# wustl-cig/FLAIR

Measured on AMD Instinct MI355X. Metric: restored frames/sec at 256x256, 16-frame clip, 250-step DDIM, higher is better.
Workload: dtype bf16

## Files before the change

### flair_amd/csrc/conv.hip

```cpp
#include <type_traits>

#include "common.h"
#include "mfma_tile.h"

namespace {

struct ConvArgs {
    const void* x[4];
    int segC[4];
    int segLd[4];
    int nseg;
    const void* w;
    const float* bias;
    const void* res0;
    const void* res1;
    int res0Ld, res1Ld;
    void* y;
    int yLd;
    int T, H, W;
    int KT, KH, KW;
    int Cout, CinTot;
    int act;
    float outScale;
    long P;
// ... 958 lines not shown
            for (int jj = 0; jj < 2; ++jj) {
                const int cofs = i * 32 + 16 * jj;
                if (tl.co0 + cofs >= a.Cout) continue;
                const bool lane_ok = tl.co0 + cofs + cl < a.Cout;
                float bv[8];
                {
                    const float4 b0 = *reinterpret_cast<const float4*>(bl + cofs);
                    const float4 b1 = *reinterpret_cast<const float4*>(bl + cofs + 4);
                    bv[0] = b0.x; bv[1] = b0.y; bv[2] = b0.z; bv[3] = b0.w; bv[4] = b1.x; bv[5] = b1.y; bv[6] = b1.z; bv[7] = b1.w;
                }
#pragma unroll
                for (int j = 0; j < RPW; ++j) {
                    float v[8];
#pragma unroll
                    for (int e = 0; e < 4; ++e) {
                        const auto sw2 = __builtin_amdgcn_permlane32_swap(__float_as_uint(acc[j][i][8 * jj + e]),
                                                                          __float_as_uint(acc[j][i][8 * jj + 4 + e]), false, false);
                        v[e] = __uint_as_float(sw2[0]) + bv[e];
                        v[4 + e] = __uint_as_float(sw2[1]) + bv[4 + e];
                    }
                    if constexpr (ACT == 0) {
#pragma unroll
                        for (int e = 0; e < 8; ++e) v[e] = fmaxf(v[e], v[e] * slope);
                    } else if constexpr (ACT == 1) {
                        dcn_offset_act<8>(v, tl.co0 + cofs + cl, a.actParam, a.actPeriod);
                    } else {
#pragma unroll
                        for (int e = 0; e < 8; ++e) v[e] = silu_f(v[e]);
                    }
                    const long ro = (long)j * W;
                    if (r0b && lane_ok) add_piece<E>(v, r0b + ro * a.res0Ld + cofs);
                    if (r1b && lane_ok) add_piece<E>(v, r1b + ro * a.res1Ld + cofs);
#pragma unroll
                    for (int e = 0; e < 8; ++e) v[e] *= scale;
                    if (!lane_ok) continue;
                    Vec16<E>::store(yb + ro * a.yLd + cofs, v);
                }
            }
    };
    auto epilogue = [&](const DmaTile& tl, int biasSlot) {
        const bool res = a.res0 || a.res1;
        auto go = [&](auto actTag) {
            if constexpr (RPW == 1) {
                epilogue_plain_as(tl, biasSlot, actTag);
            } else {
                if (res) epilogue_as(tl, biasSlot, actTag, std::true_type{});
                else epilogue_as(tl, biasSlot, actTag, std::false_type{});
            }
        };
        if (a.act == FLAIR_ACT_DCN_OFFSETS) go(std::integral_constant<int, 1>{});
        else if (a.act == FLAIR_ACT_SILU) go(std::integral_constant<int, 2>{});
        else if (RPW >= 2 && a.act == FLAIR_ACT_NONE && a.outScale == 1.f) go(std::integral_constant<int, 3>{});
        else go(std::integral_constant<int, 0>{});
    };

    DmaTile cur, nxt;
    int iCur = 0, iNxt = 0;
    if (!tile_at(0, cur)) return;
    nxt = cur;
    Walk wk;
    walk_first(nxt.t, wk);
    setup_tile(nxt);
    float4 biasReg = make_float4(0.f, 0.f, 0.f, 0.f);
    bool biasPending = false;
    auto bias_request = [&](const DmaTile& tl) {
        if (tid < 16) {
            const int bco = tl.co0 + 4 * tid;
            biasReg = (a.bias && bco < a.Cout) ? *reinterpret_cast<const float4*>(a.bias + bco) : make_float4(0.f, 0.f, 0.f, 0.f);
            if (a.fbias && bco < a.Cout) {
                const float* fb = a.fbias + (long)tl.t * a.fbiasLd + bco;
                biasReg.x += fb[0]; biasReg.y += fb[1]; biasReg.z += fb[2]; biasReg.w += fb[3];
            }
        }
        biasPending = true;
    };
    auto bias_commit = [&](int slot_) {
        if (tid < 16) *reinterpret_cast<float4*>(smem + BIAS_OFF + (slot_ & 1) * 256 + 16 * tid) = biasReg;
        biasPending = false;
    };
    bias_request(nxt);
    bias_commit(0);
    const bool res0any = a.res0 || a.res1;
    int remIssue = chunks_of(nxt.t);
    int remCompute = remIssue;
    bool more = true;
    int stage = 0;
    issue(nxt, wk, 0);
    walk_next(nxt.t, wk);
    --remIssue;
    asm volatile("s_waitcnt vmcnt(0)" ::: "memory");
    __syncthreads();
    zero_acc();
    while (true) {
        if (more && remIssue == 0) {
            ++iNxt;
            more = tile_at(iNxt, nxt);
            if (more) {
                walk_first(nxt.t, wk);
                setup_tile(nxt);
                remIssue = chunks_of(nxt.t);
                bias_request(nxt);
            }
        }
        if (more) {
            issue(nxt, wk, stage ^ 1);
            walk_next(nxt.t, wk);
            --remIssue;
        }
        compute(stage);
        if (biasPending) bias_commit(iNxt);
        bool storesInFlight = false;
        if (--remCompute == 0) {
            epilogue(cur, iCur);
            storesInFlight = RPW >= 2 ? !a.res1 : cur.co0 + 64 <= a.Cout && !res0any;
            ++iCur;
            if (!tile_at(iCur, cur)) break;
            remCompute = chunks_of(cur.t);
            zero_acc();
        }
        if (storesInFlight) {
            asm volatile("s_waitcnt vmcnt(%0)" ::"n"(4 * RPW) : "memory");
        } else {
            asm volatile("s_waitcnt vmcnt(0)" ::: "memory");
        }
        __syncthreads();
        stage ^= 1;
    }
}

template <int RPW>
__global__ __launch_bounds__(512, 2) void conv3x3_dma_kernel(ConvArgs a, int nTiles, int tilesPerXcd) {
    prefetch_kernargs<sizeof(ConvArgs) + 8>();
    conv3x3_dma_body<RPW>(a, nTiles, tilesPerXcd);
}

template <int RPW>
int launch_dma(const ConvArgs& a0, hipStream_t s) {
    constexpr int NW = 8, NSTAGE = 2, TH = NW * RPW;
    ConvArgs a = a0;
    a.nCoTiles = cdiv(a.Cout, 64);
    a.tFast = a.KT == 3 && a.T > 1;
    const int nTiles = a.T * (a.H / TH) * (a.W / 32) * a.nCoTiles;
    const int nCu = flair_cu_count();
    int grid = nTiles < nCu ? (nTiles + 7) / 8 * 8 : nCu / 8 * 8;
    if (grid < 8) grid = 8;
    const int tilesPerXcd = (nTiles + 7) / 8;
    constexpr int HALO_INSTR = ((TH + 2) * 34 + 15) / 16;
    const size_t lds = NSTAGE * (size_t)(HALO_INSTR + 36) * 1024 + NW * 1024 + 512;
    static LdsAttrOnce attr;
    {
        const hipError_t e = flair_max_lds_once(attr, reinterpret_cast<const void*>(&conv3x3_dma_kernel<RPW>));
        FLAIR_CHECK(e == hipSuccess, "flair_conv_nhwc: hipFuncSetAttribute: %s", hipGetErrorString(e));
    }
    hipLaunchKernelGGL(conv3x3_dma_kernel<RPW>, dim3(grid), dim3(64 * NW), lds, s, a, nTiles, tilesPerXcd);
    FLAIR_LAUNCH_CHECK();
    return FLAIR_OK;
}


__global__ __launch_bounds__(512, 2) void conv_frame_kernel(ConvArgs a) {
    prefetch_kernargs<sizeof(ConvArgs)>();
    using E = bf16_t;
    constexpr int NW = 8, HWP = 34;
    constexpr int HINSTR = 22, HIMG = HINSTR * 1024, WINSTR = 36, SLOT = WINSTR * 1024;
    constexpr int HR = 3, WR = 2;
    constexpr int RING = HR * HIMG, BIAS = RING + WR * SLOT;
    constexpr int NH = (HINSTR + NW - 1) / NW, NWS = (WINSTR + NW - 1) / NW;
    extern __shared__ __attribute__((aligned(16))) char smem[];
    const int tid = threadIdx.x, lane = tid & 63;
    const int wave = __builtin_amdgcn_readfirstlane(tid >> 6);
    const int lr = lane & 31, lh = lane >> 5;
    const int lrow = lane >> 2, lchunk = lane & 3;
    const int tilesW = a.W / 32, perFrame = tilesW * (a.H / 8);
    const int bid = xcd_remap(blockIdx.x, gridDim.x);
    const int t = bid / perFrame, tile = bid - t * perFrame;
    const int h0 = (tile / tilesW) * 8, w0 = (tile % tilesW) * 32;
    const int nS = a.CinTot / 32;

    const u32x4_t wdesc = make_desc(a.w, a.wBytes);
    const u32x4_t bdesc = make_desc(a.bias, a.bias ? (unsigned)a.Cout * 4u : 0u);
    dma16(bdesc, (unsigned)(lane * 16), (unsigned)BIAS);
    unsigned hpix[NH], hpiece[NH];
#pragma unroll
    for (int i = 0; i < NH; ++i) dma_halo_coords((wave * NH + i) % HINSTR, lrow, lchunk, 10, h0, w0, a.H, a.W, hpix[i], hpiece[i]);
    unsigned wlane[NWS];
#pragma unroll
    for (int i = 0; i < NWS; ++i) {
        const int id = (wave * NWS + i) % WINSTR;
        const int row = id * 16 + lrow, tap9 = row >> 6, co = row & 63;
        wlane[i] = co < a.Cout ? (unsigned)((co * 9 + tap9) * a.CinTot) * 2u + (unsigned)((lchunk ^ ((co >> 2) & 3)) << 4) : FLAIR_OOB;
    }
    int hseg = 0, hcb = 0;
    auto issue_halo = [&](int slot) {
        const unsigned ld = (unsigned)a.segLd[hseg] * 2u;
        const u32x4_t xdesc = make_desc(reinterpret_cast<const char*>(a.x[hseg]) + (size_t)t * a.H * a.W * ld, a.segBytes[hseg]);
        const unsigned cofs = (unsigned)(hcb * 64);
#pragma unroll
        for (int i = 0; i < NH; ++i) {
            const int k = (wave * NH + i) % HINSTR;
            dma16(xdesc, hpix[i] == 0xffffffffu ? FLAIR_OOB : hpix[i] * ld + cofs + hpiece[i], (unsigned)(slot * HIMG + k * 1024));
        }
        if (++hcb * 32 >= a.segC[hseg]) {
            hcb = 0;
            ++hseg;
        }
    };
    auto issue_w = [&](int s_) {
#pragma unroll
        for (int i = 0; i < NWS; ++i) {
            const int id = (wave * NWS + i) % WINSTR;
            dma16(wdesc, wlane[i] == FLAIR_OOB ? FLAIR_OOB : wlane[i] + (unsigned)(s_ * 64), (unsigned)(RING + (s_ % WR) * SLOT + id * 1024));
        }
    };
    issue_halo(0);
    issue_w(0);
    if (nS > 1) {
        issue_halo(1);
        issue_w(1);
    }
    if (nS > 2) issue_halo(2);

    unsigned aoff[2], boff[3][2];
    dma_frag_offsets(lr, lh, wave * HWP, aoff, boff);
    f32x16 acc[2];
    auto compute = [&](int wslot, int hslot) { dma_tap_loop(smem + RING + wslot * SLOT, smem + hslot * HIMG, aoff, boff, acc, dma_no_hook{}); };

    const long prow = ((long)t * a.H + h0 + wave) * a.W + w0;
    const unsigned yLdB = (unsigned)a.yLd * 2u, r0LdB = (unsigned)a.res0Ld * 2u, r1LdB = (unsigned)a.res1Ld * 2u;
    const __amdgpu_buffer_rsrc_t yd = make_rsrc(reinterpret_cast<char*>(a.y) + prow * a.yLd * 2, (unsigned)a.W * yLdB);
    const __amdgpu_buffer_rsrc_t r0d = make_rsrc(a.res0 ? reinterpret_cast<const char*>(a.res0) + prow * a.res0Ld * 2 : nullptr, a.res0 ? (unsigned)a.W * r0LdB : 0u);
    const __amdgpu_buffer_rsrc_t r1d = make_rsrc(a.res1 ? reinterpret_cast<const char*>(a.res1) + prow * a.res1Ld * 2 : nullptr, a.res1 ? (unsigned)a.W * r1LdB : 0u);
    uint4 r0v[4], r1v[4];
#pragma unroll
    for (int g = 0; g < 4; ++g) r0v[g] = r1v[g] = make_uint4(0u, 0u, 0u, 0u);

    for (int s_ = 0; s_ < nS; ++s_) {
        if (s_ + 1 >= nS) asm volatile("s_waitcnt vmcnt(0)" ::: "memory");
        else if (s_ == 0 && nS > 2) asm volatile("s_waitcnt vmcnt(%0)" ::"n"(2 * NH + NWS) : "memory");
        else if (s_ == 0) asm volatile("s_waitcnt vmcnt(%0)" ::"n"(NH + NWS) : "memory");
        else asm volatile("s_waitcnt vmcnt(%0)" ::"n"(NH) : "memory");
        __builtin_amdgcn_s_barrier();
        if (s_ == 0) {
            const float* sb = reinterpret_cast<const float*>(smem + BIAS);
#pragma unroll
            for (int cf = 0; cf < 2; ++cf)
#pragma unroll
                for (int g = 0; g < 4; ++g) {
                    const float4 bq = *reinterpret_cast<const float4*>(sb + cf * 32 + 8 * g + 4 * lh);
                    acc[cf][4 * g] = bq.x; acc[cf][4 * g + 1] = bq.y; acc[cf][4 * g + 2] = bq.z; acc[cf][4 * g + 3] = bq.w;
                }
        }
        if (s_ >= 1 && s_ + 1 < nS) issue_w(s_ + 1);
        if (s_ >= 1 && s_ + 2 < nS) issue_halo((s_ + 2) % 3);
        if (s_ + 1 == nS) {
            if (a.res0) {
#pragma unroll
                for (int g = 0; g < 4; ++g) r0v[g] = buf_load16(r0d, 16 * g + 8 * lh < a.Cout ? (unsigned)lr * r0LdB + (unsigned)(32 * g + 16 * lh) : FLAIR_OOB);
            }
            if (a.res1) {
#pragma unroll
                for (int g = 0; g < 4; ++g) r1v[g] = buf_load16(r1d, 16 * g + 8 * lh < a.Cout ? (unsigned)lr * r1LdB + (unsigned)(32 * g + 16 * lh) : FLAIR_OOB);
            }
        }
        compute(s_ % WR, s_ % HR);
    }

    const float slope = leaky_slope(a.act);
    const float scale = a.outScale;
#pragma unroll
    for (int cf = 0; cf < 2; ++cf)
#pragma unroll
        for (int jj = 0; jj < 2; ++jj) {
            const int g = 2 * cf + jj;
            float v[8];
            acc_octet(acc[cf], jj, v);
            leaky_act(v, slope);
            add_piece<E>(v, r0v[g]);
            add_piece<E>(v, r1v[g]);
#pragma unroll
            for (int e = 0; e < 8; ++e) v[e] *= scale;
            store_piece(yd, pack_piece<E>(v), 16 * g + 8 * lh < a.Cout ? (unsigned)lr * yLdB + (unsigned)(32 * g + 16 * lh) : FLAIR_OOB);
        }
}

static bool frame_kernel_ok(const ConvArgs& a) {
    if (a.esz != 2 || a.KT != 1 || a.KH != 3 || a.KW != 3 || a.stride != 1 || a.fbias || a.Cout > 64 || a.Cout % 8 || a.W % 32 || a.H % 8) return false;
    if (!(a.act == FLAIR_ACT_NONE || a.act == FLAIR_ACT_RELU || a.act == FLAIR_ACT_LRELU01 || a.act == FLAIR_ACT_LRELU02)) return false;
    if (a.tapShift || a.reflect || a.CinTot % 32 || a.CinTot < 32) return false;
    for (int i = 0; i < a.nseg; ++i)
        if (a.segC[i] % 32) return false;
    return true;
}

static int launch_frame(const ConvArgs& a, hipStream_t s) {
    constexpr size_t lds = (3 * 22 + 2 * 36) * 1024 + 1024;
    static LdsAttrOnce attr;
    const hipError_t e = flair_max_lds_once(attr, reinterpret_cast<const void*>(&conv_frame_kernel));
    FLAIR_CHECK(e == hipSuccess, "flair_conv_nhwc: hipFuncSetAttribute: %s", hipGetErrorString(e));
    hipLaunchKernelGGL(conv_frame_kernel, dim3(a.T * (a.H / 8) * (a.W / 32)), dim3(512), lds, s, a);
    FLAIR_LAUNCH_CHECK();
    return FLAIR_OK;
}

template <typename E, int TC, int TP, int WC, int WP, int PD, int KWID>
__global__ __launch_bounds__(256) void conv_igemm_kernel(ConvArgs a) {
    prefetch_kernargs<sizeof(ConvArgs)>();
    constexpr int BKE = Mma<E>::BKE * KWID;
    constexpr int ROWB = 64 * KWID;
    constexpr int CPR = 4 * KWID;
    constexpr int RPP = 256 / CPR;
    constexpr int VEC = ET<E>::VEC;
    constexpr int FC = TC / WC / 32;
    constexpr int FP = TP / WP / 32;
    constexpr int XR = TP / RPP;
    constexpr int WR = TC / RPP;
    static_assert(WC * WP == 4 && FC >= 1 && FP >= 1 && XR >= 1 && WR >= 1, "tile");

    extern __shared__ __attribute__((aligned(16))) char smem[];
    constexpr int BUF = (TC + TP) * ROWB;
    auto loff = [](int row, int chunk) { return KWID == 1 ? lds_off(row, chunk) : row * 128 + ((chunk ^ ((row >> 1) & 7)) << 4); };

    const int tid = threadIdx.x;
    const int lane = tid & 63, wave = __builtin_amdgcn_readfirstlane(tid >> 6);
    const int wc = wave / WP, wp = wave % WP;

    const int bid = xcd_remap(blockIdx.x, gridDim.x);
    const int coTile = bid % a.nCoTiles;
    const int pixTile = bid / a.nCoTiles;
    const long p0 = (long)pixTile * TP;
    const int co0 = coTile * TC;

    const int chunk = tid % CPR;
    const int srow = tid / CPR;
    int xt[XR], xh[XR], xw[XR];
    bool xvalid[XR];
#pragma unroll
    for (int i = 0; i < XR; ++i) {
        long p = p0 + srow + RPP * i;
        xvalid[i] = p < a.P;
        if (!xvalid[i]) p = 0;
        int w_ = (int)(p % a.W);
        long q = p / a.W;
        xw[i] = w_;
        xh[i] = (int)(q % a.H);
        xt[i] = (int)(q / a.H);
    }
    const int taps = a.KT * a.KH * a.KW;
    const int pt = a.KT / 2, ph = a.KH / 2, pw = a.KW / 2;
    const int tFirst = (int)(p0 / ((long)a.H * a.W));
    const int tileFrames = (int)((TP + (long)a.H * a.W - 1) / ((long)a.H * a.W)) + 1;

    uint4 xreg[PD][XR], wreg[PD][WR];

    const int nkAll = taps * (a.CinTot / BKE);
    const int ks0 = (int)((long)blockIdx.y * nkAll / a.splitK);
    const int ks1 = (int)((long)(blockIdx.y + 1) * nkAll / a.splitK);
    int tap = ks0 / (a.CinTot / BKE), seg = 0, cb = ks0 % (a.CinTot / BKE), segOff = 0;
    while (cb * BKE >= a.segC[seg]) {
        cb -= a.segC[seg] / BKE;
        segOff += a.segC[seg];
        ++seg;
    }
    int dw = tap % a.KW - pw, dh = (tap / a.KW) % a.KH - ph, dt = tap / (a.KW * a.KH) - pt;

    const __amdgpu_buffer_rsrc_t wrs = make_rsrc(a.w, a.wBytes);
    constexpr unsigned ESZ = sizeof(E);
    auto issue_loads = [&](int set) {
        const int ld = a.segLd[seg];
        int fb = tFirst + dt;
        fb = fb < 0 ? 0 : (fb >= a.T ? a.T - 1 : fb);
        int nfr = a.T - fb;
        if (nfr > tileFrames) nfr = tileFrames;
        const size_t frameBytes = (size_t)a.Hin * a.Win * ld * ESZ;
        const __amdgpu_buffer_rsrc_t xr =
            make_rsrc(reinterpret_cast<const char*>(a.x[seg]) + fb * frameBytes, (unsigned)(nfr * frameBytes));
        const int coff = cb * BKE + chunk * VEC;
#pragma unroll
        for (int i = 0; i < XR; ++i) {
            const int t2 = xt[i] + dt;
            int h2 = xh[i] * a.stride + dh + a.tapShift, w2 = xw[i] * a.stride + dw + a.tapShift;
            if (a.reflect) {
                h2 = h2 < 0 ? -h2 : (h2 >= a.Hin ? 2 * a.Hin - 2 - h2 : h2);
                w2 = w2 < 0 ? -w2 : (w2 >= a.Win ? 2 * a.Win - 2 - w2 : w2);
            }
            const bool ok = xvalid[i] && (unsigned)t2 < (unsigned)a.T && (unsigned)h2 < (unsigned)a.Hin &&
                            (unsigned)w2 < (unsigned)a.Win;
            const unsigned off = ok ? (unsigned)((((t2 - fb) * a.Hin + h2) * a.Win + w2) * ld + coff) * ESZ : FLAIR_OOB;
            xreg[set][i] = buf_load16(xr, off);
        }
        const unsigned kofs = (unsigned)(tap * a.CinTot + segOff + coff) * ESZ;
#pragma unroll
        for (int j = 0; j < WR; ++j) {
            const int n = co0 + srow + RPP * j;
            wreg[set][j] = buf_load16(wrs, n < a.Cout ? (unsigned)(n * taps * a.CinTot) * ESZ + kofs : FLAIR_OOB);
        }
    };
    auto advance = [&]() {
        ++cb;
        if (cb * BKE >= a.segC[seg]) {
            cb = 0;
            segOff += a.segC[seg];
            ++seg;
            if (seg >= a.nseg) {
                seg = 0;
                segOff = 0;
                ++tap;
                ++dw;
                if (dw > pw) {
                    dw = -pw;
                    ++dh;
                    if (dh > ph) {
                        dh = -ph;
                        ++dt;
                    }
                }
            }
        }
    };
    auto write_lds = [&](int buf, int set) {
        char* base = smem + buf * BUF;
#pragma unroll
        for (int j = 0; j < WR; ++j)
            *reinterpret_cast<uint4*>(base + loff(srow + RPP * j, chunk)) = wreg[set][j];
#pragma unroll
        for (int i = 0; i < XR; ++i)
            *reinterpret_cast<uint4*>(base + TC * ROWB + loff(srow + RPP * i, chunk)) = xreg[set][i];
    };

    f32x16 acc[FC][FP];
#pragma unroll
    for (int i = 0; i < FC; ++i)
#pragma unroll
        for (int j = 0; j < FP; ++j)
#pragma unroll
            for (int r = 0; r < 16; ++r) acc[i][j][r] = 0.f;

    const int nk = ks1 - ks0;
    const int lr = lane & 31, lh = lane >> 5;

#pragma unroll
    for (int u = 0; u < PD; ++u)
        if (u < nk) {
            issue_loads(u);
            advance();
        }
    write_lds(0, 0);
    __syncthreads();

    for (int ks = 0; ks < nk; ks += PD) {
#pragma unroll
        for (int u = 0; u < PD; ++u) {
            const int k = ks + u;
            if (k >= nk) break;
            const int cur = k & 1;
            if (k + PD < nk) {
                issue_loads(u);
                advance();
            }
            const char* wb = smem + cur * BUF;
            const char* xb = wb + TC * ROWB;
#pragma unroll
            for (int sp = 0; sp < KWID; ++sp) {
                uint4 af[FC][2], bfr[FP][2];
#pragma unroll
                for (int i = 0; i < FC; ++i) {
                    const int row = wc * (TC / WC) + i * 32 + lr;
                    af[i][0] = *reinterpret_cast<const uint4*>(wb + loff(row, 4 * sp + Mma<E>::chunk(0, lh)));
                    af[i][1] = *reinterpret_cast<const uint4*>(wb + loff(row, 4 * sp + Mma<E>::chunk(1, lh)));
                }
#pragma unroll
                for (int j = 0; j < FP; ++j) {
                    const int row = wp * (TP / WP) + j * 32 + lr;
                    bfr[j][0] = *reinterpret_cast<const uint4*>(xb + loff(row, 4 * sp + Mma<E>::chunk(0, lh)));
                    bfr[j][1] = *reinterpret_cast<const uint4*>(xb + loff(row, 4 * sp + Mma<E>::chunk(1, lh)));
                }
#pragma unroll
                for (int i = 0; i < FC; ++i)
#pragma unroll
                    for (int j = 0; j < FP; ++j) Mma<E>::run(af[i], bfr[j], acc[i][j]);
            }
            if (k + 1 < nk) write_lds(cur ^ 1, (u + 1) % PD);
            __syncthreads();
        }
    }

    if (a.splitK > 1) {
#pragma unroll
        for (int j = 0; j < FP; ++j) {
            const long p = p0 + wp * (TP / WP) + j * 32 + lr;
            if (p >= a.P) continue;
#pragma unroll
            for (int i = 0; i < FC; ++i)
#pragma unroll
                for (int g = 0; g < 4; ++g) {
                    const int co = co0 + wc * (TC / WC) + i * 32 + 8 * g + 4 * lh;
                    if (co < a.Cout)
                        *reinterpret_cast<float4*>(a.part + ((long)blockIdx.y * a.P + p) * a.Cout + co) =
                            make_float4(acc[i][j][4 * g], acc[i][j][4 * g + 1], acc[i][j][4 * g + 2],
                                        acc[i][j][4 * g + 3]);
                }
        }
        return;
    }
    if ((a.Cout & 7) == 0 && ((uintptr_t)a.y & 15) == 0 && (a.yLd * (int)sizeof(E)) % 16 == 0 &&
        (!a.res0 || (((uintptr_t)a.res0 & 15) == 0 && (a.res0Ld * (int)sizeof(E)) % 16 == 0)) &&
        (!a.res1 || (((uintptr_t)a.res1 & 15) == 0 && (a.res1Ld * (int)sizeof(E)) % 16 == 0))) {
        auto run = [&](auto actTag) {
            igemm_epilogue<E, decltype(actTag)::value, FC, FP>(a, acc, p0 + wp * (TP / WP), co0 + wc * (TC / WC), lr, lh);
        };
        if (a.act == FLAIR_ACT_DCN_OFFSETS) run(std::integral_constant<int, 1>{});
        else if (a.act == FLAIR_ACT_SILU) run(std::integral_constant<int, 2>{});
        else if (a.act == FLAIR_ACT_GELU) run(std::integral_constant<int, 3>{});
        else run(std::integral_constant<int, 0>{});
        return;
    }
#pragma unroll
    for (int j = 0; j < FP; ++j) {
        const long p = p0 + wp * (TP / WP) + j * 32 + lr;
        if (p >= a.P) continue;
#pragma unroll
        for (int i = 0; i < FC; ++i)
#pragma unroll
            for (int g = 0; g < 4; ++g)
                store_quad<E>(a, p, co0 + wc * (TC / WC) + i * 32 + 8 * g + 4 * lh, acc[i][j][4 * g],
                              acc[i][j][4 * g + 1], acc[i][j][4 * g + 2], acc[i][j][4 * g + 3]);
    }
}

template <typename E>
__global__ void conv_splitk_reduce_kernel(ConvArgs a) {
    const unsigned cq = (unsigned)(a.Cout / 4);
    const unsigned quads = (unsigned)a.P * cq;
    const size_t slice = (size_t)a.P * a.Cout;
    for (unsigned i = blockIdx.x * blockDim.x + threadIdx.x; i < quads; i += gridDim.x * blockDim.x) {
        const unsigned p = i / cq;
        const int co = (int)(i - p * cq) * 4;
        const float* src = a.part + (size_t)p * a.Cout + co;
        float4 s = make_float4(0.f, 0.f, 0.f, 0.f);
        int k = 0;
        for (; k + 4 <= a.splitK; k += 4) {
            float4 v[4];
#pragma unroll
            for (int u = 0; u < 4; ++u) v[u] = *reinterpret_cast<const float4*>(src + (size_t)(k + u) * slice);
#pragma unroll
            for (int u = 0; u < 4; ++u) {
                s.x += v[u].x; s.y += v[u].y; s.z += v[u].z; s.w += v[u].w;
            }
        }
        for (; k < a.splitK; ++k) {
            const float4 v = *reinterpret_cast<const float4*>(src + (size_t)k * slice);
            s.x += v.x; s.y += v.y; s.z += v.z; s.w += v.w;
        }
        store_quad<E>(a, p, co, s.x, s.y, s.z, s.w);
    }
}

template <typename E, int TC, int TP, int WC, int WP, int PD, int KWID>
int launch_pd(const ConvArgs& a0, hipStream_t s) {
    ConvArgs a = a0;
    a.nPixTiles = cdiv(a.P, TP);
    a.nCoTiles = cdiv(a.Cout, TC);
    const int grid = a.nPixTiles * a.nCoTiles;
    const size_t lds = 2 * (TC + TP) * 64 * KWID;
    hipLaunchKernelGGL((conv_igemm_kernel<E, TC, TP, WC, WP, PD, KWID>), dim3(grid, a.splitK), dim3(256), lds, s, a);
    FLAIR_LAUNCH_CHECK();
    if (a.splitK > 1) {
        hipLaunchKernelGGL(conv_splitk_reduce_kernel<E>, dim3(grid_for(a.P * (a.Cout / 4), 256, 2048)), dim3(256), 0, s, a);
        FLAIR_LAUNCH_CHECK();
    }
    return FLAIR_OK;
}

template <typename E, int TC, int TP, int WC, int WP>
int launch(const ConvArgs& a, hipStream_t s) {
    if constexpr (sizeof(E) == 2) {
        bool ok = true;
        for (int i = 0; i < a.nseg; ++i) ok = ok && a.segC[i] % 64 == 0;
        if (ok) return launch_pd<E, TC, TP, WC, WP, 2, 2>(a, s);
    }
    return launch_pd<E, TC, TP, WC, WP, 4, 1>(a, s);
}

enum ConvVariant {
    IGEMM_128x128 = 0,
    IGEMM_64x128 = 1,
    IGEMM_64x64 = 2,
    HALO_8 = 3,
    HALO_4 = 4,
    HALO_2 = 5,
    HALO_KS_8 = 6,
    HALO_KS_4 = 7,
    DMA_CLIP = 8,
    DMA_FRAME = 9,
};

int choose_split(const ConvArgs& a, ConvVariant variant) {
    if (variant > IGEMM_64x64) return 1;
    const int maxBlocks = variant == IGEMM_128x128 ? 512 : 1024, maxSplit = 16;
    const int tc = variant == IGEMM_128x128 ? 128 : 64, tp = variant == IGEMM_64x64 ? 64 : 128;
    const int bke = 64 / (a.wBytes && a.CinTot ? (int)(a.wBytes / ((unsigned long long)a.Cout * a.KT * a.KH * a.KW * a.CinTot)) : 2);
    const long nk = (long)a.KT * a.KH * a.KW * (a.CinTot / bke);
    const long tiles = (long)cdiv(a.P, tp) * cdiv(a.Cout, tc);
    if (tiles >= 384 || nk < 32) return 1;
    long s = maxBlocks / tiles;
    if (s > maxSplit) s = maxSplit;
    if (s > nk / 8) s = nk / 8;
    return s < 1 ? 1 : (int)s;
}

ConvVariant choose_variant(const ConvArgs& a) {
    if (!a.reflect && a.stride == 1 && a.KH == 3 && a.KW == 3 && a.W % 32 == 0 && a.H >= 2) {
        const long per = (long)a.T * (a.W / 32) * cdiv(a.Cout, 64);
        const bool ks = a.Cout % 8 == 0;
        if (a.esz == 2 && ks && a.act != FLAIR_ACT_GELU && a.H % 16 == 0 && per * cdiv(a.H, 8) > 256 && per * (a.H / 16) >= 192) return DMA_CLIP;
        const bool dmaOk = a.esz == 2 && ks && a.act != FLAIR_ACT_GELU;
        if (per * cdiv(a.H, 8) >= 256) return ks && per * cdiv(a.H, 8) <= 256 ? (dmaOk && a.H % 8 == 0 ? DMA_FRAME : HALO_KS_8) : HALO_8;
        if (per * cdiv(a.H, 4) >= 256) return ks && per * cdiv(a.H, 4) <= 256 ? HALO_KS_4 : HALO_4;
        return HALO_2;
    }
    const long tiles128 = (long)cdiv(a.P, 128) * cdiv(a.Cout, 128);
    if (a.Cout > 64 && tiles128 >= 512) return IGEMM_128x128;
    if (a.Cout >= 128 && a.P >= 1024 && tiles128 <= 64 && (long)a.KT * a.KH * a.KW * a.CinTot >= 2304) return IGEMM_128x128;
    const long tiles64x128 = (long)cdiv(a.P, 128) * cdiv(a.Cout, 64);
    if (tiles64x128 >= 512) return IGEMM_64x128;
    return IGEMM_64x64;
}

template <typename E>
int dispatch(const ConvArgs& a0, hipStream_t s) {
    ConvArgs a = a0;
    const ConvVariant variant = choose_variant(a);
    a.splitK = a.part ? choose_split(a, variant) : 1;
    switch (variant) {
        case IGEMM_128x128: return launch<E, 128, 128, 2, 2>(a, s);
        case IGEMM_64x128: return launch<E, 64, 128, 1, 4>(a, s);
        case IGEMM_64x64: return launch<E, 64, 64, 2, 2>(a, s);
        case HALO_8: return launch_halo<E, 8>(a, s);
        case HALO_4: return launch_halo<E, 4>(a, s);
        case HALO_KS_8: return launch_halo_ks<E, 8>(a, s);
        case HALO_KS_4: return launch_halo_ks<E, 4>(a, s);
        case DMA_CLIP: return launch_dma<2>(a, s);
        case DMA_FRAME:
            if (frame_kernel_ok(a)) return launch_frame(a, s);
            return launch_dma<1>(a, s);
        case HALO_2: break;
    }
    return launch_halo<E, 2>(a, s);
}

}

extern "C" int flair_conv_variant(const flair_conv_params* p);

static void fill_geometry(ConvArgs& a, const flair_conv_params* p) {
    a.stride = p->stride > 1 ? p->stride : 1;
    a.Hin = p->H; a.Win = p->W;
    a.T = p->T; a.KT = p->KT; a.KH = p->KH; a.KW = p->KW; a.Cout = p->Cout;
    a.reflect = p->reflect_pad ? 1 : 0;
    a.act = p->act;
    a.H = (p->H + a.stride - 1) / a.stride;
    a.W = (p->W + a.stride - 1) / a.stride;
    a.P = (long)p->T * a.H * a.W;
    a.CinTot = 0;
    for (int i = 0; i < p->nseg && i < 4; ++i) a.CinTot += p->seg_c[i];
    const int esz = p->dtype == FLAIR_BF16 ? 2 : 4;
    a.esz = esz;
    a.wBytes = (unsigned)((unsigned long long)p->Cout * p->KT * p->KH * p->KW * a.CinTot * esz);
}

extern "C" size_t flair_conv_workspace_bytes(const flair_conv_params* p) {
    if (!p) return 0;
    ConvArgs a{};
    fill_geometry(a, p);
    const int split = choose_split(a, choose_variant(a));
    return split > 1 ? (size_t)split * a.P * a.Cout * sizeof(float) : 0;
}

extern "C" int flair_conv_nhwc(const flair_conv_params* p, const void* const* x, const void* w,
                               const float* bias, const float* frame_bias, const void* res0, const void* res1,
                               void* y, void* workspace, size_t workspace_bytes, hipStream_t stream) {
    FLAIR_CHECK(p && x && w && y, "flair_conv_nhwc: null argument");
    FLAIR_CHECK_DTYPE("flair_conv_nhwc", p->dtype);
    FLAIR_CHECK(p->nseg >= 1 && p->nseg <= 4, "flair_conv_nhwc: nseg %d not in 1..4", p->nseg);
    FLAIR_CHECK(p->T > 0 && p->H > 0 && p->W > 0 && p->Cout > 0, "flair_conv_nhwc: empty shape");
    FLAIR_CHECK((p->KT & 1) && (p->KH & 1) && (p->KW & 1), "flair_conv_nhwc: kernel taps must be odd");
    FLAIR_CHECK(p->Cout % 4 == 0, "flair_conv_nhwc: Cout %d must be a multiple of 4", p->Cout);
    const int bke = p->dtype == FLAIR_BF16 ? 32 : 16;
    const int esz = p->dtype == FLAIR_BF16 ? 2 : 4;
    ConvArgs a{};
    fill_geometry(a, p);
    for (int i = 0; i < p->nseg; ++i) {
        FLAIR_CHECK(x[i], "flair_conv_nhwc: segment %d is null", i);
        FLAIR_CHECK(p->seg_c[i] > 0 && p->seg_c[i] % bke == 0,
                    "flair_conv_nhwc: segment %d has %d channels; must be a multiple of %d", i, p->seg_c[i], bke);
        FLAIR_CHECK(p->seg_ld[i] >= p->seg_c[i] && (p->seg_ld[i] * esz) % 16 == 0 &&
                        ((uintptr_t)x[i]) % 16 == 0,
                    "flair_conv_nhwc: segment %d stride/alignment", i);
        a.x[i] = x[i];
        a.segC[i] = p->seg_c[i];
        a.segLd[i] = p->seg_ld[i];
        const unsigned long long bytes = (unsigned long long)p->H * p->W * p->seg_ld[i] * esz;
        FLAIR_CHECK(bytes < 0x40000000ull, "flair_conv_nhwc: one frame of segment %d spans %llu bytes (limit 1 GiB)",
                    i, bytes);
        a.segBytes[i] = (unsigned)bytes;
    }
    {
        const unsigned long long wb = (unsigned long long)p->Cout * p->KT * p->KH * p->KW * a.CinTot * esz;
        FLAIR_CHECK(wb < 0x80000000ull, "flair_conv_nhwc: weights span %llu bytes (limit 2 GiB)", wb);
    }
    const int gran = (p->dtype == FLAIR_BF16 && p->Cout % 8 != 0) ? 8 : 16;
    FLAIR_CHECK(p->y_ld >= p->Cout && (p->y_ld * esz) % gran == 0 && ((uintptr_t)y) % 16 == 0,
                "flair_conv_nhwc: output stride/alignment (y_ld = %d: >= Cout = %d, a multiple of %d bytes; y 16-byte aligned)",
                p->y_ld, p->Cout, gran);
    FLAIR_CHECK(!res0 || (p->res_ld[0] >= p->Cout && (p->res_ld[0] * esz) % gran == 0 && ((uintptr_t)res0) % gran == 0),
                "flair_conv_nhwc: res0 stride/alignment (res_ld = %d: >= Cout = %d; stride and pointer multiples of %d bytes)",
                p->res_ld[0], p->Cout, gran);
    FLAIR_CHECK(!res1 || (p->res_ld[1] >= p->Cout && (p->res_ld[1] * esz) % gran == 0 && ((uintptr_t)res1) % gran == 0),
                "flair_conv_nhwc: res1 stride/alignment (res_ld = %d: >= Cout = %d; stride and pointer multiples of %d bytes)",
                p->res_ld[1], p->Cout, gran);
    FLAIR_CHECK(((uintptr_t)w) % 16 == 0, "flair_conv_nhwc: weight alignment");
    FLAIR_CHECK(!bias || ((uintptr_t)bias) % 16 == 0, "flair_conv_nhwc: bias alignment");
    a.nseg = p->nseg;
    a.w = w;
    a.bias = bias;
    a.fbias = frame_bias;
    a.fbiasLd = p->frame_bias_ld;
    FLAIR_CHECK(!frame_bias || p->frame_bias_ld >= p->Cout, "flair_conv_nhwc: frame_bias_ld");
    {
        const unsigned long long hw = (unsigned long long)p->H * p->W * esz;
        FLAIR_CHECK(hw * p->y_ld < 0x40000000ull && (!res0 || hw * p->res_ld[0] < 0x40000000ull) && (!res1 || hw * p->res_ld[1] < 0x40000000ull),
                    "flair_conv_nhwc: one frame of the output / a residual spans more than 1 GiB");
    }
    a.res0 = res0;
    a.res1 = res1;
    a.res0Ld = p->res_ld[0];
    a.res1Ld = p->res_ld[1];
    a.y = y;
    a.yLd = p->y_ld;
    a.actParam = p->act_param;
    a.actPeriod = p->act_period;
    FLAIR_CHECK(p->act != FLAIR_ACT_DCN_OFFSETS || (p->act_period > 0 && p->act_period % 24 == 0),
                "flair_conv_nhwc: FLAIR_ACT_DCN_OFFSETS needs act_period = 3 * deform_groups (multiple of 24), got %d",
                p->act_period);
    a.outScale = p->out_scale;
    FLAIR_CHECK(a.stride == 1 || a.stride == 2, "flair_conv_nhwc: stride %d unsupported", p->stride);
    FLAIR_CHECK(!p->asym_pad || (a.stride == 2 && a.KH == a.KW && a.KT == 1 && p->H % 2 == 0 && p->W % 2 == 0),
                "flair_conv_nhwc: asym_pad needs a square 2-D stride-2 kernel on even frames");
    a.tapShift = p->asym_pad ? a.KH / 2 : 0;
    FLAIR_CHECK(!p->reflect_pad || (!p->asym_pad && a.KT == 1 && p->H > a.KH / 2 && p->W > a.KW / 2),
                "flair_conv_nhwc: reflect_pad needs a 2-D kernel smaller than the frame");
    a.part = nullptr;
    a.splitK = 1;

    const size_t need = flair_conv_workspace_bytes(p);
    if (workspace && need > 0 && workspace_bytes >= need) {
        FLAIR_CHECK(((uintptr_t)workspace) % 16 == 0, "flair_conv_nhwc: workspace alignment");
        a.part = reinterpret_cast<float*>(workspace);
    }
    if (p->dtype == FLAIR_BF16) return dispatch<bf16_t>(a, stream);
    return dispatch<float>(a, stream);
}

extern "C" int flair_conv_variant(const flair_conv_params* p) {
    if (!p) return -1;
    ConvArgs a{};
    fill_geometry(a, p);
    return choose_variant(a);
}
```

Measured before the change: 0.8652.

## Add intra-workgroup K-group split to implicit-GEMM conv with LDS reduction

Adds a KG template parameter so one workgroup runs 256*KG threads, each 256-thread group handling its own slice of the K loop in separate LDS staging buffers. The partial accumulators are then reduced through LDS before the epilogue. A new plan function picks KG=2 for 128x128 tiles and KG=4 for 64x64 tiles in bf16, cutting the cross-block split-K factor and with it the fp32 workspace traffic and reduce kernel. The change also raises the K threshold for the small-tile 128x128 path in bf16. The cost is more LDS per workgroup, which can lower occupancy, plus extra barriers and an LDS reduction step.

```diff
diff --git a/flair_amd/csrc/conv.hip b/flair_amd/csrc/conv.hip
--- a/flair_amd/csrc/conv.hip
+++ b/flair_amd/csrc/conv.hip
@@ -1284,8 +1284,9 @@
     return FLAIR_OK;
 }
 
-template <typename E, int TC, int TP, int WC, int WP, int PD, int KWID>
-__global__ __launch_bounds__(256) void conv_igemm_kernel(ConvArgs a) {
+template <typename E, int TC, int TP, int WC, int WP, int PD, int KWID, int KG>
+__global__ __launch_bounds__(256 * KG) void conv_igemm_kernel(ConvArgs a) {
+    static_assert(KG == 1 || KG == 2 || KG == 4, "K groups");
     prefetch_kernargs<sizeof(ConvArgs)>();
     constexpr int BKE = Mma<E>::BKE * KWID;
     constexpr int ROWB = 64 * KWID;
@@ -1302,9 +1303,11 @@
     constexpr int BUF = (TC + TP) * ROWB;
     auto loff = [](int row, int chunk) { return KWID == 1 ? lds_off(row, chunk) : row * 128 + ((chunk ^ ((row >> 1) & 7)) << 4); };
 
-    const int tid = threadIdx.x;
+    const int tid = KG == 1 ? threadIdx.x : threadIdx.x & 255;
+    const int kgrp = KG == 1 ? 0 : __builtin_amdgcn_readfirstlane(threadIdx.x >> 8);
     const int lane = tid & 63, wave = __builtin_amdgcn_readfirstlane(tid >> 6);
     const int wc = wave / WP, wp = wave % WP;
+    char* const gmem = KG == 1 ? smem : smem + kgrp * (2 * BUF);
 
     const int bid = xcd_remap(blockIdx.x, gridDim.x);
     const int coTile = bid % a.nCoTiles;
@@ -1335,8 +1338,11 @@
     uint4 xreg[PD][XR], wreg[PD][WR];
 
     const int nkAll = taps * (a.CinTot / BKE);
-    const int ks0 = (int)((long)blockIdx.y * nkAll / a.splitK);
-    const int ks1 = (int)((long)(blockIdx.y + 1) * nkAll / a.splitK);
+    const int by0 = (int)((long)blockIdx.y * nkAll / a.splitK);
+    const int by1 = (int)((long)(blockIdx.y + 1) * nkAll / a.splitK);
+    const int gtrips = (by1 - by0 + KG - 1) / KG;
+    const int ks0 = KG == 1 ? by0 : (by0 + kgrp * gtrips < by1 ? by0 + kgrp * gtrips : by1);
+    const int ks1 = KG == 1 ? by1 : (ks0 + gtrips < by1 ? ks0 + gtrips : by1);
     int tap = ks0 / (a.CinTot / BKE), seg = 0, cb = ks0 % (a.CinTot / BKE), segOff = 0;
     while (cb * BKE >= a.segC[seg]) {
         cb -= a.segC[seg] / BKE;
@@ -1400,7 +1406,7 @@
         }
     };
     auto write_lds = [&](int buf, int set) {
-        char* base = smem + buf * BUF;
+        char* base = gmem + buf * BUF;
 #pragma unroll
         for (int j = 0; j < WR; ++j)
             *reinterpret_cast<uint4*>(base + loff(srow + RPP * j, chunk)) = wreg[set][j];
@@ -1418,6 +1424,7 @@
             for (int r = 0; r < 16; ++r) acc[i][j][r] = 0.f;
 
     const int nk = ks1 - ks0;
+    const int trips = KG == 1 ? nk : gtrips;
     const int lr = lane & 31, lh = lane >> 5;
 
 #pragma unroll
@@ -1426,21 +1433,22 @@
             issue_loads(u);
             advance();
         }
-    write_lds(0, 0);
+    if (KG == 1 || nk > 0) write_lds(0, 0);
     __syncthreads();
 
-    for (int ks = 0; ks < nk; ks += PD) {
+    for (int ks = 0; ks < trips; ks += PD) {
 #pragma unroll
         for (int u = 0; u < PD; ++u) {
             const int k = ks + u;
-            if (k >= nk) break;
+            if (k >= trips) break;
             const int cur = k & 1;
             if (k + PD < nk) {
                 issue_loads(u);
                 advance();
             }
-            const char* wb = smem + cur * BUF;
+            const char* wb = gmem + cur * BUF;
             const char* xb = wb + TC * ROWB;
+            if (KG == 1 || k < nk)
 #pragma unroll
             for (int sp = 0; sp < KWID; ++sp) {
                 uint4 af[FC][2], bfr[FP][2];
@@ -1464,6 +1472,33 @@
             if (k + 1 < nk) write_lds(cur ^ 1, (u + 1) % PD);
             __syncthreads();
         }
+    }
+
+    if constexpr (KG > 1) {
+        float4* red = reinterpret_cast<float4*>(smem);
+        if (kgrp > 0) {
+#pragma unroll
+            for (int i = 0; i < FC; ++i)
+#pragma unroll
+                for (int j = 0; j < FP; ++j)
+#pragma unroll
+                    for (int q = 0; q < 4; ++q)
+                        red[(((kgrp - 1) * FC * FP + i * FP + j) * 4 + q) * 256 + tid] =
+                            make_float4(acc[i][j][4 * q], acc[i][j][4 * q + 1], acc[i][j][4 * q + 2], acc[i][j][4 * q + 3]);
+        }
+        __syncthreads();
+        if (kgrp > 0) return;
+#pragma unroll
+        for (int g = 1; g < KG; ++g)
+#pragma unroll
+            for (int i = 0; i < FC; ++i)
+#pragma unroll
+                for (int j = 0; j < FP; ++j)
+#pragma unroll
+                    for (int q = 0; q < 4; ++q) {
+                        const float4 v = red[(((g - 1) * FC * FP + i * FP + j) * 4 + q) * 256 + tid];
+                        acc[i][j][4 * q] += v.x; acc[i][j][4 * q + 1] += v.y; acc[i][j][4 * q + 2] += v.z; acc[i][j][4 * q + 3] += v.w;
+                    }
     }
 
     if (a.splitK > 1) {
@@ -1537,14 +1572,21 @@
     }
 }
 
-template <typename E, int TC, int TP, int WC, int WP, int PD, int KWID>
+template <typename E, int TC, int TP, int WC, int WP, int PD, int KWID, int KG>
 int launch_pd(const ConvArgs& a0, hipStream_t s) {
     ConvArgs a = a0;
     a.nPixTiles = cdiv(a.P, TP);
     a.nCoTiles = cdiv(a.Cout, TC);
     const int grid = a.nPixTiles * a.nCoTiles;
-    const size_t lds = 2 * (TC + TP) * 64 * KWID;
-    hipLaunchKernelGGL((conv_igemm_kernel<E, TC, TP, WC, WP, PD, KWID>), dim3(grid, a.splitK), dim3(256), lds, s, a);
+    constexpr size_t staging = (size_t)KG * 2 * (TC + TP) * 64 * KWID, sums = (size_t)(KG - 1) * TC * TP * 4;
+    constexpr size_t lds = staging > sums ? staging : sums;
+    static_assert(lds <= 160 * 1024, "one workgroup's LDS");
+    if constexpr (lds > 64 * 1024) {
+        static LdsAttrOnce attr;
+        const hipError_t e = flair_max_lds_once(attr, reinterpret_cast<const void*>(&conv_igemm_kernel<E, TC, TP, WC, WP, PD, KWID, KG>));
+        FLAIR_CHECK(e == hipSuccess, "flair_conv_nhwc: hipFuncSetAttribute: %s", hipGetErrorString(e));
+    }
+    hipLaunchKernelGGL((conv_igemm_kernel<E, TC, TP, WC, WP, PD, KWID, KG>), dim3(grid, a.splitK), dim3(256 * KG), lds, s, a);
     FLAIR_LAUNCH_CHECK();
     if (a.splitK > 1) {
         hipLaunchKernelGGL(conv_splitk_reduce_kernel<E>, dim3(grid_for(a.P * (a.Cout / 4), 256, 2048)), dim3(256), 0, s, a);
@@ -1553,14 +1595,14 @@
     return FLAIR_OK;
 }
 
-template <typename E, int TC, int TP, int WC, int WP>
+template <typename E, int TC, int TP, int WC, int WP, int KG = 1>
 int launch(const ConvArgs& a, hipStream_t s) {
     if constexpr (sizeof(E) == 2) {
         bool ok = true;
         for (int i = 0; i < a.nseg; ++i) ok = ok && a.segC[i] % 64 == 0;
-        if (ok) return launch_pd<E, TC, TP, WC, WP, 2, 2>(a, s);
-    }
-    return launch_pd<E, TC, TP, WC, WP, 4, 1>(a, s);
+        if (ok) return launch_pd<E, TC, TP, WC, WP, 2, 2, KG>(a, s);
+    }
+    return launch_pd<E, TC, TP, WC, WP, 4, 1, KG>(a, s);
 }
 
 enum ConvVariant {
@@ -1602,17 +1644,41 @@
     }
     const long tiles128 = (long)cdiv(a.P, 128) * cdiv(a.Cout, 128);
     if (a.Cout > 64 && tiles128 >= 512) return IGEMM_128x128;
-    if (a.Cout >= 128 && a.P >= 1024 && tiles128 <= 64 && (long)a.KT * a.KH * a.KW * a.CinTot >= 2304) return IGEMM_128x128;
+    const long K = (long)a.KT * a.KH * a.KW * a.CinTot;
+    if (a.Cout >= 128 && a.P >= 1024 && tiles128 <= 64 && K >= (a.esz == 2 ? 4608 : 2304)) return IGEMM_128x128;
     const long tiles64x128 = (long)cdiv(a.P, 128) * cdiv(a.Cout, 64);
     if (tiles64x128 >= 512) return IGEMM_64x128;
     return IGEMM_64x64;
+}
+
+struct SplitPlan {
+    int kg, split;
+};
+
+SplitPlan choose_plan(const ConvArgs& a, ConvVariant variant) {
+    const int s0 = choose_split(a, variant);
+    if (s0 <= 1 || a.esz != 2) return {1, s0};
+    const long nk = (long)a.KT * a.KH * a.KW * (a.CinTot / 32);
+    if (variant == IGEMM_128x128) return nk <= 288 ? SplitPlan{2, (s0 + 1) / 2} : SplitPlan{1, s0};
+    if (variant != IGEMM_64x64) return {1, s0};
+    const long tiles = (long)cdiv(a.P, 64) * cdiv(a.Cout, 64);
+    const int kg = 4;
+    int split = 1;
+    if (nk / (2 * kg) > 8)
+        while (tiles * split < 256 && split < 16 && nk / (2 * kg * split * 2) >= 2) split *= 2;
+    return {kg, split};
 }
 
 template <typename E>
 int dispatch(const ConvArgs& a0, hipStream_t s) {
     ConvArgs a = a0;
     const ConvVariant variant = choose_variant(a);
-    a.splitK = a.part ? choose_split(a, variant) : 1;
+    const SplitPlan plan = choose_plan(a, variant);
+    a.splitK = a.part ? plan.split : 1;
+    if constexpr (sizeof(E) == 2) {
+        if (variant == IGEMM_128x128 && plan.kg == 2) return launch<E, 128, 128, 2, 2, 2>(a, s);
+        if (variant == IGEMM_64x64 && plan.kg == 4) return launch<E, 64, 64, 2, 2, 4>(a, s);
+    }
     switch (variant) {
         case IGEMM_128x128: return launch<E, 128, 128, 2, 2>(a, s);
         case IGEMM_64x128: return launch<E, 64, 128, 1, 4>(a, s);
@@ -1654,7 +1720,7 @@
     if (!p) return 0;
     ConvArgs a{};
     fill_geometry(a, p);
-    const int split = choose_split(a, choose_variant(a));
+    const int split = choose_plan(a, choose_variant(a)).split;
     return split > 1 ? (size_t)split * a.P * a.Cout * sizeof(float) : 0;
 }
 
```

After: 0.8674 (median of 6 runs). Within noise of the previous version (+0.3%).
